# DassHydro-dev/smash

Measured on AMD Instinct MI355X. Metric: cell-timesteps/s, forward+adjoint sweep, higher is better.
Workload: dtype f32

## Files before the change

### __graft_entry__.py

```python
from __future__ import annotations

import os
import subprocess
import sys

ROOT = os.path.dirname(os.path.abspath(__file__))
if ROOT not in sys.path:
    sys.path.insert(0, ROOT)

HIPCC = os.environ.get("HIPCC", "/opt/rocm/bin/hipcc")
CSRC = os.path.join(ROOT, "smash_amd", "csrc")
LIB = os.path.join(ROOT, "smash_amd", "libsmashx.so")
LIB_EXACT = os.path.join(ROOT, "smash_amd", "libsmashx_exact.so")
HIP_FLAGS = ["-O3", "-ffp-contract=off", "--offload-arch=gfx950", "-fPIC", "-shared", "-std=c++17"]


def _newer(target, sources):
    if not os.path.exists(target):
        return False
    t = os.path.getmtime(target)
    return all(os.path.getmtime(s) <= t for s in sources)


def build() -> None:
    srcs = [os.path.join(CSRC, f) for f in sorted(os.listdir(CSRC)) if f.endswith((".hip", ".cpp", ".h"))]
    srcs += [os.path.join(ROOT, "include", "smashx.h"), os.path.join(ROOT, "include", "smashx_setup.h"),
             os.path.join(ROOT, "include", "smashx_forcing.h"), os.path.join(ROOT, "include", "smashx_prcp.h"),
             os.path.join(ROOT, "include", "smashx_signature.h"), os.path.join(ROOT, "include", "smashx_hyper.h"),
             os.path.join(ROOT, "include", "smashx_ann.h"), os.path.join(ROOT, "include", "smashx_sbs.h")]
    jobs = []
    for lib, extra in ((LIB, []), (LIB_EXACT, ["-DSX_EXACT_LIBM=1"])):
        if not _newer(lib, srcs):
            cmd = [HIPCC] + HIP_FLAGS + extra + ["-pthread", "-o", lib, os.path.join(CSRC, "smashx.hip"), os.path.join(CSRC, "sx_plan.cpp"),
                                                 os.path.join(CSRC, "sx_lbfgsb.cpp"), os.path.join(CSRC, "sx_hyper.cpp"), os.path.join(CSRC, "sx_sbs.cpp")]
            jobs.append((cmd, subprocess.Popen(cmd, cwd=ROOT)))
    for cmd, j in jobs:
        if j.wait() != 0:
            raise subprocess.CalledProcessError(j.returncode, cmd)
    subprocess.check_call(["make", "-s", "-C", os.path.join(ROOT, "oracle"), "liboracle.so", "liboracle64.so"])
    ref_src = os.environ.get("SMASH_REFERENCE", "/root/reference")
    ref_lib = os.path.join(ROOT, "oracle", "_ref", "libsmash_ref.so")
    dropin = os.path.join(ROOT, "oracle", "_ref", "libsmash_dropin.so")
    shim = [os.path.join(ROOT, "fortran", "smashx_dropin.f90"), os.path.join(ROOT, "fortran", "smashx_setulb.f90"),
            os.path.join(ROOT, "include", "smashx.h"), os.path.join(ROOT, "oracle", "ref", "ref_capi.f90"),
            os.path.join(ROOT, "oracle", "ref", "build_ref.sh")]
    native_lb = os.path.join(ROOT, "oracle", "_ref", "libsmash_dropin_lbfgsb.so")
    if os.path.isdir(os.path.join(ref_src, "smash", "solver")) and not (os.path.exists(ref_lib) and _newer(dropin, shim) and _newer(native_lb, shim)):
        subprocess.check_call(["bash", os.path.join(ROOT, "oracle", "ref", "build_ref.sh")])
    import smash_amd
    from smash_amd import _lib
    L = _lib.lib()
    missing = [s for s in _lib.SYMBOLS + _lib.SETUP_SYMBOLS + _lib.FORCING_SYMBOLS + _lib.PRCP_SYMBOLS + _lib.SIGNATURE_SYMBOLS + _lib.HYPER_DEVICE_SYMBOLS + _lib.ANN_SYMBOLS + _lib.SBS_SYMBOLS if not hasattr(L, s)]
    if missing:
        raise RuntimeError(f"libsmashx.so lacks {missing}")


def smoke() -> None:
    import numpy as np

    sys.path.insert(0, os.path.join(ROOT, "tests"))
    import golden_util as gu

    import smash_amd
    from oracle import pyoracle
    if not os.path.exists(LIB):
        build()
    g = gu.load("gr_b_16x16x96_nse_gaps")
    ref = pyoracle.run(g.structure, g.mesh, g.dt, g.prcp, g.pet, g.qobs, g.params, g.states, adjoint=True, **g.opts)
    for k, v in g.adj["parameters_b"].items():
        assert np.array_equal(ref["parameters_b"][k], v), k

    setup = smash_amd.SetupDT(0, g.mesh.ng, structure=g.structure, dt=g.dt, ntime_step=g.nt)
    setup.optimize.jobs_fun, setup.optimize.wjobs_fun = ["nse"], [1.0]
    mesh = smash_amd.MeshDT.from_synth(setup, g.mesh)
    inp = smash_amd.Input_DataDT(setup, mesh)
    inp.prcp, inp.pet, inp.qobs = g.prcp, g.pet, g.qobs
    par = smash_amd.ParametersDT.from_dict(mesh, g.params)
    sta = smash_amd.StatesDT.from_dict(mesh, g.states)
    out = smash_amd.OutputDT(setup, mesh)
    par_b, sta_b = par.copy(), sta.copy()
    smash_amd.forward_b(setup, mesh, inp, par, par_b, par.copy(), par.copy(), sta, sta_b, sta.copy(), sta.copy(), out,
                        out.copy(), np.float32(0), np.float32(1))

    errs = {"qsim": (gu.rel_l2(out.qsim, ref["qsim"]), gu.tol(g.noise["qsim"].max())),
            "cost": (abs(out.cost - ref["cost"]), gu.tol_cost(g.noise["cost"], ref["cost"]))}
# ... 15 lines not shown
```

### include/smashx.h

```cpp
#ifndef SMASHX_H
#define SMASHX_H

#ifdef __cplusplus
extern "C" {
#endif

#define SMASHX_GNP 16
#define SMASHX_GNS 8

enum { SMASHX_GR_A = 1, SMASHX_GR_B = 2, SMASHX_GR_C = 3, SMASHX_GR_D = 4, SMASHX_VIC_A = 5 };
enum { SMASHX_NSE = 1, SMASHX_KGE = 2, SMASHX_KGE2 = 3, SMASHX_SE = 4, SMASHX_RMSE = 5, SMASHX_LOGARITHMIC = 6,
       SMASHX_CRC = 7, SMASHX_CFP2 = 8, SMASHX_CFP10 = 9, SMASHX_CFP50 = 10, SMASHX_CFP90 = 11, SMASHX_EPF = 12, SMASHX_ELT = 13,
       SMASHX_ERC = 14 };
enum { SMASHX_PRIOR = 1, SMASHX_SMOOTHING = 2, SMASHX_HARD_SMOOTHING = 3 };
enum { SMASHX_P_CI = 0, SMASHX_P_CP = 1, SMASHX_P_BETA = 2, SMASHX_P_CFT = 3, SMASHX_P_CST = 4, SMASHX_P_ALPHA = 5,
       SMASHX_P_EXC = 6, SMASHX_P_B = 7, SMASHX_P_CUSL1 = 8, SMASHX_P_CUSL2 = 9, SMASHX_P_CLSL = 10, SMASHX_P_KS = 11,
       SMASHX_P_DS = 12, SMASHX_P_DSM = 13, SMASHX_P_WS = 14, SMASHX_P_LR = 15 };
enum { SMASHX_S_HI = 0, SMASHX_S_HP = 1, SMASHX_S_HFT = 2, SMASHX_S_HST = 3, SMASHX_S_HUSL1 = 4, SMASHX_S_HUSL2 = 5,
       SMASHX_S_HLSL = 6, SMASHX_S_HLR = 7 };

enum {
    SMASHX_OK = 0,
    SMASHX_E_ARG = -1,
    SMASHX_E_UNSUPPORTED = -2,
// ... 177 lines not shown
    SMASHX_FN_POW_M025 = 9,
    SMASHX_FN_POW_M025_M125 = 10,
    SMASHX_FN_POW_3P5 = 11,
    SMASHX_FN_POW_3P5_2P5 = 12,
    SMASHX_FN_DIV = 13,
    SMASHX_FN_DIV4 = 14,
    SMASHX_FN_FDIV = 15,
    SMASHX_FN_DIV_FAST = 16,
    SMASHX_FN_COUNT = 17
};
int smashx_selftest_eval(int device, int fn, const float* x, const float* y, long long n, float* out0, float* out1);

#define SMASHX_LBFGSB_START 0
#define SMASHX_LBFGSB_FG 1
#define SMASHX_LBFGSB_NEW_X 2
#define SMASHX_LBFGSB_CONVERGED 3
#define SMASHX_LBFGSB_ABNORMAL 4
typedef struct smashx_lbfgsb smashx_lbfgsb;
int smashx_lbfgsb_create(long n, int m, const double* lower, const double* upper, double factr, double pgtol, smashx_lbfgsb** out);
int smashx_lbfgsb_step(smashx_lbfgsb* opt, double* x, double f, const double* g, int* task);
long smashx_lbfgsb_iterations(const smashx_lbfgsb* opt);
long smashx_lbfgsb_evaluations(const smashx_lbfgsb* opt);
double smashx_lbfgsb_projected_gradient(const smashx_lbfgsb* opt);
const char* smashx_lbfgsb_message(const smashx_lbfgsb* opt);
int smashx_lbfgsb_destroy(smashx_lbfgsb* opt);

#include "smashx_setup.h"
#include "smashx_forcing.h"
#include "smashx_prcp.h"
#include "smashx_signature.h"
#include "smashx_hyper.h"
#include "smashx_ann.h"
#include "smashx_sbs.h"

#ifdef __cplusplus
}
#endif
#endif
```

### smash_amd/_lib.py

```python
from __future__ import annotations

import ctypes as C
import os

_HERE = os.path.dirname(os.path.abspath(__file__))
EXACT = os.environ.get("SMASHX_EXACT_LIBM", "0") not in ("", "0")
LIB_PATH = os.environ.get("SMASHX_LIB", os.path.join(_HERE, "libsmashx_exact.so" if EXACT else "libsmashx.so"))

ABI_VERSION = 9
GNP, GNS = 16, 8
E_OK, E_ARG, E_UNSUPPORTED, E_HIP, E_NODEVICE, E_MESH, E_STATE = 0, -1, -2, -3, -4, -5, -6
STRUCTURES = {"gr-a": 1, "gr-b": 2, "gr-c": 3, "gr-d": 4, "vic-a": 5}
JOBS_FUN = {"nse": 1, "kge": 2, "kge2": 3, "se": 4, "rmse": 5, "logarithmic": 6,
            "Crc": 7, "Cfp2": 8, "Cfp10": 9, "Cfp50": 10, "Cfp90": 11, "Epf": 12, "Elt": 13, "Erc": 14}
SIGNATURE_FUN = ("Crc", "Cfp2", "Cfp10", "Cfp50", "Cfp90", "Epf", "Elt", "Erc")
JREG_FUN = {"prior": 1, "smoothing": 2, "hard_smoothing": 3}
HYPER = {"hyper-linear": 1, "hyper-polynomial": 2}
LBFGSB_START, LBFGSB_FG, LBFGSB_NEW_X, LBFGSB_CONVERGED, LBFGSB_ABNORMAL = range(5)
COMM_ID_BYTES = 128
FN = {k: i for i, k in enumerate("TANH TANH_BRANCHY EXPM1 EXP LOG POW POWB POW_M4 POW_M4_M5 POW_M025 POW_M025_M125 POW_3P5 POW_3P5_2P5 "
                                 "DIV DIV4 FDIV DIV_FAST".split())}
FN_COUNT = len(FN)

HALO_FN = C.CFUNCTYPE(C.c_int, C.c_void_p, C.c_int, C.c_int, C.c_int)
# ... 145 lines not shown
HYPER_DEVICE_SYMBOLS = list(HYPER_DEVICE_PROTOTYPES)
ANN_LAYER = {"dense": 1, "relu": 2, "leaky_relu": 3, "elu": 4, "selu": 5, "sigmoid": 6, "tanh": 7, "scale": 8,
             "softplus": 9, "softmax": 10, "dropout": 11}
_graph = [_int, _int, ptr, ptr, _int]
ANN_PROTOTYPES = {
    "smashx_ann_set_descriptors": (_int, [ptr, _int, ptr]),
    "smashx_ann_set_net": (_int, [ptr, _int, ptr, ptr, _int, ptr, ptr, ptr]),
    "smashx_ann_upload": (_int, [ptr, ptr]),
    "smashx_ann_gradient": (_int, [ptr, ptr]),
    "smashx_ann_fields": (_int, [ptr, _par, _sta]),
    "smashx_ann_info": (_int, [ptr, ptr, ptr]),
    "smashx_ann_host_nweights": (_int, _graph),
    "smashx_ann_host_forward": (_int, _graph + [ptr, ptr, ptr, _long, ptr, ptr]),
    "smashx_ann_host_gradient": (_int, _graph + [ptr, ptr, ptr, _long, ptr, ptr, ptr]),
    "smashx_ann_host_activation": (_int, [_int, _long, ptr, ptr, ptr]),
    "smashx_ann_host_exp": (_int, [_long, ptr, ptr]),
}
ANN_SYMBOLS = list(ANN_PROTOTYPES)
SBS_PROTOTYPES = {
    "smashx_sbs_create": (_int, [_int, ptr, ptr, ptr, _float, _int, _out]),
    "smashx_sbs_ask": (_int, [ptr, ptr, ptr]),
    "smashx_sbs_tell": (_int, [ptr, ptr]),
    "smashx_sbs_x": (_int, [ptr, ptr]),
    "smashx_sbs_gx": (_float, [ptr]),
    "smashx_sbs_ddx": (_float, [ptr]),
    "smashx_sbs_iter": (_int, [ptr]),
    "smashx_sbs_nfg": (_int, [ptr]),
    "smashx_sbs_message": (_str, [ptr]),
    "smashx_sbs_destroy": (_int, [ptr]),
    "smashx_uniform_costs": (_int, [ptr, _par, _sta, _int, ptr, ptr, _int, ptr]),
    "smashx_uniform_costs_info": (_int, [ptr, ptr, ptr]),
}
SBS_SYMBOLS = list(SBS_PROTOTYPES)


class SmashxError(RuntimeError):
    def __init__(self, code, msg):
        super().__init__(f"libsmashx error {code}: {msg}")
        self.code = code


_lib = None


def lib():
    global _lib
    if _lib is None:
        if not os.path.exists(LIB_PATH):
            raise ImportError(f"{LIB_PATH} is missing: build the HIP library first (__graft_entry__.build()); "
                              "smash_amd has no CPU fallback")
        L = C.CDLL(LIB_PATH)
        for name, (restype, argtypes) in list(PROTOTYPES.items()) + list(SETUP_PROTOTYPES.items()) + list(FORCING_PROTOTYPES.items()) + list(PRCP_PROTOTYPES.items()) + list(SIGNATURE_PROTOTYPES.items()) + list(HYPER_DEVICE_PROTOTYPES.items()) + list(ANN_PROTOTYPES.items()) + list(SBS_PROTOTYPES.items()):
            fn = getattr(L, name)
            fn.restype, fn.argtypes = restype, argtypes
        sizes = (C.c_int * 7)()
        L.smashx_abi_sizes(sizes)
        mine = [C.sizeof(t) for t in (Config, Mesh, Options, Parameters, States, Costs, Timing)]
        if list(sizes) != mine:
            raise ImportError(f"{LIB_PATH} was built from another include/smashx.h (struct sizes {list(sizes)}, this module expects {mine}): "
                              "rebuild it (__graft_entry__.build())")
        _lib = L
    return _lib


def check(rc):
    if rc != 0:
        raise SmashxError(rc, lib().smashx_last_error().decode())
```

### smash_amd/csrc/smashx.hip

```cpp
#include "../../include/smashx.h"

#include <hip/hip_runtime.h>
#include <rccl/rccl.h>

#include <dlfcn.h>

#include <algorithm>
#include <functional>
#include <numeric>
#include <cstdio>
#include <cstdlib>
#include <cstring>
#include <string>
#include <vector>

#include "sx_cost.h"
#include "sx_jreg.h"
#include "sx_kernels.h"
#include "sx_ensemble.h"
#include "sx_resident.h"
#include "sx_fields.h"
#include "sx_interception.h"
#include "sx_meanforcing.h"
#include "sx_prcpindices.h"
// ... 248 lines not shown
        if (r_ != ncclSuccess)                                                                          \
            return fail(SMASHX_E_HIP, std::string(#expr) + ": " + rccl().GetErrorString(r_) + " (" + __FILE__ + ":" + std::to_string(__LINE__) + ")"); \
    } while (0)

struct SxComm {
    ncclComm_t comm = nullptr;
    int rank = 0, nranks = 1, device = -1;
    hipStream_t stream = nullptr;
    double* d_buf = nullptr;
    std::vector<smashx_plan*> plans;
};
struct PeerSeg { int rank, first, count; };

struct Launch { hipEvent_t a, b; int kind; double cellsteps; };

}

struct smashx_plan {
    smashx_config cfg{};
    SxSchedule sch;
    int n = 0, npad = 0, nt = 0, ng = 0, st = 0;
    long n2 = 0;
    int M = 0;
    int Tc = 0, nchunks = 0;
    bool have_forcing = false, have_options = false, have_qobs = false, uploaded = false;
    bool chunk_ready = false, adj_ready = false;
    smashx_options opt{};
    std::vector<float> wgauge;
    std::vector<int> gauge_flwacc_h;
    hipStream_t stream = nullptr;
    hipStream_t stream_r = nullptr;
    int Tp = 0;
    bool hi_tape = true;
    int chain_from = 1;
    bool chain_stage = false; SxStageTables stg{}; int stg_blocks = 0, stg_rows_extra = 0; size_t stg_lds = 0;
    float* hrk = nullptr; bool hrk_tried = false, early_adj = true;
    size_t vlds_fwd = 0, vlds_adj = 0;
    std::vector<hipEvent_t> buf_free;
    std::vector<double> round_ncells;
    bool chain_used = false;
    bool chain = true;
    int n_out = 0, n_in = 0;
    int *d_out_x = nullptr, *d_in_x = nullptr;
    float *halo_out = nullptr, *halo_in = nullptr;
    smashx_halo_fn halo_fn = nullptr; void* halo_user = nullptr;
    SxComm* xcomm = nullptr;
    std::vector<PeerSeg> out_segs, in_segs;
    int *d_out_xp = nullptr, *d_in_xp = nullptr;
    float *x_out = nullptr, *x_in = nullptr;
    float* x_keep = nullptr; size_t x_keep_cap = 0;
    std::vector<void*> allocs; std::vector<size_t> alloc_bytes;
    double bytes = 0;
    double hbm_free_at_plan = -1.0, hbm_total = -1.0;
    SxDeviceArrays A{};
    int* d_cell_flat = nullptr;
    int* d_sparse_idx = nullptr;
    float last_jobs_d = 0.f, last_jreg_d = 0.f;
    long n_sparse = 0;
    float* d_stage = nullptr;
    long stage_planes = 0;
    float* d_full[SX_NFIELDS] = {nullptr};
    float* st0[SX_NSSLOTS] = {nullptr};
    float* ckpt = nullptr;
    float* d_prcp = nullptr; float* d_pet = nullptr;
    int* d_ctrl_pos = nullptr; double* d_ctrl = nullptr; size_t ctrl_cap = 0;
    smashx_forcing_layout flay{};
// ... 219 lines not shown
        p->A.hr_rows = Tc / 4;
        p->A.nx = std::max(p->sch.nxslots, 1);
        p->nchunks = (p->nt + Tc - 1) / Tc;
        {
            int want = p->cfg.pipe_steps > 0 ? p->cfg.pipe_steps : Tc;
            const int nsub = std::max(1, (Tc + want / 2) / want);
            p->Tp = std::min(Tc, ((Tc + nsub - 1) / nsub + 15) / 16 * 16);
        }
        int rc;
        if ((rc = p->dmalloc(&p->A.qtT, (size_t)p->npad * Tc))) return rc;
        if ((rc = p->dmalloc(&p->A.xT, (size_t)std::max(p->sch.nxslots, 1) * Tc))) return rc;
        HIPCHK(hipMemsetAsync(p->A.qtT, 0, (size_t)p->npad * Tc * 4, p->stream));
        HIPCHK(hipMemsetAsync(p->A.xT, 0, (size_t)std::max(p->sch.nxslots, 1) * Tc * 4, p->stream));
        p->chunk_ready = true;
    }
    if (p->h_qsim_domain && !p->A.qdT) {
        int rc;
        if ((rc = p->dmalloc(&p->A.qdT, (size_t)p->npad * p->Tc))) return rc;
    }
    if (adjoint && !p->adj_ready) {
        int rc;
        const size_t cs = (size_t)p->npad * p->Tc;
        if (p->A.qsk) { p->dfree(p->A.qsk); p->A.qsk = nullptr; }
        {
            const char* e = getenv("SMASHX_HR_SKEW");
            p->A.hr_skew = e ? atoi(e) != 0 : true;
            if ((rc = p->dmalloc(&p->A.hrT, cs))) return rc;
        }
        if ((rc = p->dmalloc(&p->A.tape_hp, cs))) return rc;
        if ((rc = p->dmalloc(&p->A.tape_hft, cs))) return rc;
        if (st == 5 || ((st == 2 || st == 3) && p->hi_tape)) { if ((rc = p->dmalloc(&p->A.tape_hi, cs))) return rc; }
        else if (st == 2 || st == 3) { if ((rc = p->dmalloc(&p->A.ckpt_hi, cs / SX_HIK))) return rc; }
        if (st == 3) { if ((rc = p->dmalloc(&p->A.tape_hst, cs))) return rc; }
        if (p->nchunks > 1) { if ((rc = p->dmalloc(&p->ckpt, (size_t)p->nchunks * SX_NSSLOTS * p->npad))) return rc; }
        for (int s = 0; s < SX_NSLOTS; ++s) if ((rc = p->dmalloc(&slot_vecs(p, s).grad, (size_t)p->npad))) return rc;
        if ((rc = p->dmalloc(&p->A.qgb, (size_t)std::max(p->ngc, 1) * p->nt))) return rc;
        if ((rc = p->dmalloc(&p->d_qsim_b, (size_t)std::max(p->ng, 1) * p->nt))) return rc;
        p->adj_ready = true;
    }
    if (p->A.ncs > 0 && !p->A.qsk) {
        const size_t need = (size_t)p->A.ncs * 16 * ((size_t)p->Tc / 4 + p->stg_rows_extra + 1);
        size_t fr = 0, tot = 0;
        HIPCHK(hipMemGetInfo(&fr, &tot));
        if ((double)fr > (double)need + 2.0e9) { int rc; if ((rc = p->dmalloc(&p->A.qsk, need / 4))) return rc; }
    }
    if (adjoint && !p->hrk_tried) {
        p->hrk_tried = true;
        const int cf = chain_first(p);
        const char* e = getenv("SMASHX_KEEP_CHAIN_TAPE");
        const bool want = e ? atoi(e) != 0 : true;
        if (const char* ea = getenv("SMASHX_EARLY_ADJ_CHAIN")) p->early_adj = atoi(ea) != 0;
        if (want && p->nchunks > 1 && cf < p->sch.nrounds && !p->tiled && p->n_in == 0 && p->n_out == 0 && p->Tp >= p->Tc) {
            const int kcs0 = p->sch.g_slot_begin[p->sch.round_group_begin[cf]], kncs = p->sch.nslots - kcs0;
            const size_t need = (size_t)(p->nchunks - 1) * (size_t)(p->Tc / 4) * (size_t)kncs * 16;
            size_t fr = 0, tot = 0;
            HIPCHK(hipMemGetInfo(&fr, &tot));
            if (kncs > 0 && (double)fr > (double)need + 2.0e9) {
                int rc; if ((rc = p->dmalloc(&p->hrk, need / 4))) return rc;
                p->A.kcs0 = kcs0; p->A.kncs = kncs;
            }
        }
    }
    return 0;
}

SxDeviceArrays view_at(const smashx_plan* p, int off) {
    SxDeviceArrays B = p->A;
    B.k0 = 0; B.k1 = p->n;
    const size_t q = (size_t)(off / 4);
    B.qtT = p->A.qtT + q * p->npad * 4;
    B.hrk = nullptr;
    if (p->A.hrT) { if (p->A.hr_skew) B.hr_row0 = (int)q; else B.hrT = p->A.hrT + q * p->npad * 4; }
    if (p->A.qdT) B.qdT = p->A.qdT + q * p->npad * 4;
    if (!p->chain) B.qsk = nullptr;
    B.xT = p->A.xT + q * p->A.nx * 4;
    if (p->A.qtdT) B.qtdT = p->A.qtdT + q * p->npad * 4;
    if (p->A.xdT) B.xdT = p->A.xdT + q * p->A.nx * 4;
    if (p->A.tape_hp) B.tape_hp = p->A.tape_hp + (size_t)off * p->npad;
    if (p->A.tape_hft) B.tape_hft = p->A.tape_hft + (size_t)off * p->npad;
    if (p->A.tape_hi) B.tape_hi = p->A.tape_hi + (size_t)off * p->npad;
    if (p->A.ckpt_hi) B.ckpt_hi = p->A.ckpt_hi + (size_t)(off / SX_HIK) * p->npad;
    if (p->A.tape_hst) B.tape_hst = p->A.tape_hst + (size_t)off * p->npad;
    return B;
}

typedef void (*VertKernel)(SxDeviceArrays, int, int);
VertKernel vert_fwd_kernel(int st, bool tape, bool compact) {
#define SX_GR(ST) {sx_k_vert_fwd<ST, false, false>, sx_k_vert_fwd<ST, false, true>, sx_k_vert_fwd<ST, true, false>, sx_k_vert_fwd<ST, true, true>}
    static const VertKernel k[5][4] = {SX_GR(1), SX_GR(2), SX_GR(3), SX_GR(4),
                                       {sx_k_vert_fwd_vic<false, false>, sx_k_vert_fwd_vic<false, true>, sx_k_vert_fwd_vic<true, false>, sx_k_vert_fwd_vic<true, true>}};
#undef SX_GR
    return k[st - 1][2 * tape + compact];
}
VertKernel vert_adj_kernel(int st, bool compact) {
    static const VertKernel k[5][2] = {{sx_k_vert_adj<1, false>, sx_k_vert_adj<1, true>}, {sx_k_vert_adj<2, false>, sx_k_vert_adj<2, true>},
                                       {sx_k_vert_adj<3, false>, sx_k_vert_adj<3, true>}, {sx_k_vert_adj<4, false>, sx_k_vert_adj<4, true>},
                                       {sx_k_vert_adj_vic<false>, sx_k_vert_adj_vic<true>}};
    return k[st - 1][compact];
}
VertKernel vert_tan_kernel(int st) {
    static const VertKernel k[5] = {sx_k_vert_fwd_d<1>, sx_k_vert_fwd_d<2>, sx_k_vert_fwd_d<3>, sx_k_vert_fwd_d<4>, sx_k_vert_fwd_vic_d};
    return k[st - 1];
}
void launch_vert(smashx_plan* p, VertKernel k, int kind, size_t lds, int off, int t0, int T) {
    const SxDeviceArrays B = view_at(p, off);
    if (B.k1 <= B.k0) return;
    const dim3 grid((B.k1 - B.k0 + SX_VBLOCK - 1) / SX_VBLOCK), block(SX_VBLOCK);
    p->mark_begin(kind, p->stream, (double)(B.k1 - B.k0) * T);
    hipLaunchKernelGGL(k, grid, block, lds, p->stream, B, t0, T);
    p->mark_end();
}
void vert_fwd(smashx_plan* p, int off, bool tape, int t0, int T) {
    launch_vert(p, vert_fwd_kernel(p->st, tape, p->A.prcp16 != nullptr), 0, p->st == 5 ? 0 : p->vlds_fwd, off, t0, T);
}
void vert_adj(smashx_plan* p, int off, int t0, int T) {
    launch_vert(p, vert_adj_kernel(p->st, p->A.prcp16 != nullptr), 3, p->st == 5 ? 0 : p->vlds_adj, off, t0, T);
}
void vert_tan(smashx_plan* p, int off, int t0, int T) { launch_vert(p, vert_tan_kernel(p->st), 0, 0, off, t0, T); }
double round_cells(const smashx_plan* p, int r0, int r1) {
    double c = 0.0;
    for (int r = r0; r < r1; ++r) c += p->round_ncells[r];
    return c;
}
int chain_first(const smashx_plan* p) {
    const int nr = p->sch.nrounds;
    return (p->chain && nr - p->chain_from >= 2) ? p->chain_from : nr;
}
void reset_chain_counters(smashx_plan* p, hipStream_t st) {
    (void)hipMemsetAsync(p->A.prog, 0, (size_t)p->sch.ngroups * sizeof(int), st);
    (void)hipMemsetAsync(p->A.prog + p->sch.ngroups + 1, 0, sizeof(int), st);
}
void route_fwd_rounds(smashx_plan* p, int off, bool tape, int t0, int T, hipStream_t st, int r0, int r1, int tan = 0) {
    SxDeviceArrays B = view_at(p, off);
    if (!p->dom_q_active) B.qdT = nullptr;
    if (tan) B.qsk = nullptr;
    const size_t lds = (size_t)2 * p->M * sizeof(float4);
    void (*const k)(SxDeviceArrays, int, int, int, int) = tan == 1 ? sx_k_route_fwd<true, false, 1> : tan == 2 ? sx_k_route_fwd<false, false, 2>
                                                         : tape ? sx_k_route_fwd<true, false> : sx_k_route_fwd<false, false>;
    for (int r = r0; r < r1; ++r) {
        const int g0 = p->sch.round_group_begin[r], ngr = p->sch.round_group_begin[r + 1] - g0;
        p->mark_begin(1, st, round_cells(p, r, r + 1) * T);
        hipLaunchKernelGGL(k, dim3(ngr), dim3(p->M), lds, st, B, g0, g0 + ngr, t0, T);
        p->mark_end();
    }
}
// ... 1358 lines not shown
                                     tiled ? cfg->tile : nullptr, sch, mesh->owner_mask, sublevels_env());
    if (rc) return fail(rc == -5 ? SMASHX_E_MESH : SMASHX_E_ARG, sch.error);
    const int no = (int)sch.out_x.size(), ni = (int)sch.in_x.size();
    const int v[8] = {sch.n, sch.nrounds, sch.ngroups, sch.nslots, sch.nxslots, sch.max_stage, no, ni};
    for (int i = 0; i < 8; ++i) info[i] = v[i];
    if (no > cap || ni > cap) { if (out_src || in_src) return fail(SMASHX_E_ARG, "edge capacity too small"); return 0; }
    for (int i = 0; i < no; ++i) { if (out_src) out_src[i] = sch.out_src[i]; if (out_dst) out_dst[i] = sch.out_dst[i]; }
    for (int i = 0; i < ni; ++i) { if (in_src) in_src[i] = sch.in_src[i]; if (in_dst) in_dst[i] = sch.in_dst[i]; }
    return 0;
}

int smashx_halo_counts(const smashx_plan* p, int* n_out, int* n_in) {
    if (!p || !n_out || !n_in) return fail(SMASHX_E_ARG, "null argument");
    *n_out = p->n_out; *n_in = p->n_in;
    return 0;
}

int smashx_halo_edges(const smashx_plan* p, int* out_src, int* out_dst, int* in_src, int* in_dst) {
    if (!p) return fail(SMASHX_E_ARG, "null plan");
    for (int i = 0; i < p->n_out; ++i) { if (out_src) out_src[i] = p->sch.out_src[i]; if (out_dst) out_dst[i] = p->sch.out_dst[i]; }
    for (int i = 0; i < p->n_in; ++i) { if (in_src) in_src[i] = p->sch.in_src[i]; if (in_dst) in_dst[i] = p->sch.in_dst[i]; }
    return 0;
}

int smashx_plan_chunking(smashx_plan* p, int* chunk_steps, int* pipe_steps) {
    if (!p) return fail(SMASHX_E_ARG, "null plan");
    int rc = set_device(p); if (rc) return rc;
    if ((rc = ensure_chunk_buffers(p, true))) return rc;
    if (chunk_steps) *chunk_steps = p->Tc;
    if (pipe_steps) *pipe_steps = p->Tp;
    return 0;
}

int smashx_plan_hbm(const smashx_plan* p, double out[3]) {
    if (!p || !out) return fail(SMASHX_E_ARG, "null argument");
    out[0] = p->hbm_free_at_plan; out[1] = p->hbm_total; out[2] = p->bytes;
    return 0;
}

int smashx_set_halo(smashx_plan* p, float* d_out_buf, float* d_in_buf, smashx_halo_fn fn, void* user) {
    if (!p) return fail(SMASHX_E_ARG, "null plan");
    if (fn && ((p->n_out > 0 && !d_out_buf) || (p->n_in > 0 && !d_in_buf))) return fail(SMASHX_E_ARG, "halo buffers missing");
    p->halo_out = d_out_buf; p->halo_in = d_in_buf; p->halo_fn = fn; p->halo_user = user;
    return 0;
}

int smashx_set_median_slots(smashx_plan* p, int nslots, const int* slot_of_gauge, smashx_reduce_fn fn, void* user) {
    if (!p || nslots < 0 || (nslots > 0 && !slot_of_gauge)) return fail(SMASHX_E_ARG, "bad argument");
    int rc = set_device(p); if (rc) return rc;
    p->med_nslots = 0; p->med_fn = fn; p->med_user = user;
    if (nslots == 0) return 0;
    std::vector<int> sl(std::max(p->ng, 1), -1);
    for (int g = 0; g < p->ng; ++g) {
        sl[g] = slot_of_gauge[g];
        if (sl[g] < -1 || sl[g] >= nslots) return fail(SMASHX_E_ARG, "slot_of_gauge out of range");
    }
    if (p->have_qobs)
        for (int g = 0; g < p->ng; ++g) {
            if (!(p->wgauge[g] < 0.f) || sl[g] < 0 || gauge_has_data(p, p->h_qobs, g, p->opt.optimize_start_step - 1)) continue;
            return fail(SMASHX_E_UNSUPPORTED, "gauge " + std::to_string(g + 1) + " is given a median slot and has no qobs >= 0 from optimize_start_step on");
        }
    if (p->d_med_slot) { p->dfree(p->d_med_slot); p->dfree(p->d_medx); p->dfree(p->d_medx_idx); }
    if ((rc = p->upload_vec(&p->d_med_slot, sl))) return rc;
    p->med_slot_h = sl;
    if ((rc = p->dmalloc(&p->d_medx, (size_t)3 * nslots))) return rc;
    if ((rc = p->dmalloc(&p->d_medx_idx, (size_t)nslots))) return rc;
// ... 1243 lines not shown
```

### smash_amd/csrc/sx_kernels.h

```cpp
#pragma once

#include <hip/hip_runtime.h>

#include <climits>

#include "sx_ops.h"
#include "sx_tangent.h"
#include "sx_vic.h"

#define SX_BT 4
#define SX_VBLOCK 256

__device__ __forceinline__ void sx_lds_barrier() {
    __builtin_amdgcn_fence(__ATOMIC_RELEASE, "workgroup", "local");
    __builtin_amdgcn_s_barrier();
    __builtin_amdgcn_fence(__ATOMIC_ACQUIRE, "workgroup", "local");
}

__device__ __forceinline__ void sx_lds_wave_fence() {
    __builtin_amdgcn_fence(__ATOMIC_RELEASE, "workgroup", "local");
    __builtin_amdgcn_wave_barrier();
    __builtin_amdgcn_fence(__ATOMIC_ACQUIRE, "workgroup", "local");
}

// ... 80 lines not shown
            }
            __builtin_amdgcn_s_sleep(32);
        }
    }
    __builtin_amdgcn_fence(__ATOMIC_ACQUIRE, "agent");
}
__device__ __forceinline__ void sx_publish(int* prog, int blocks) {
    __builtin_amdgcn_fence(__ATOMIC_RELEASE, "agent");
    __hip_atomic_store((sx_gint*)prog, blocks, __ATOMIC_RELAXED, __HIP_MEMORY_SCOPE_AGENT);
}

struct SxDeviceArrays {
    int n, npad, nt, Tc;
    int k0, k1;
    int nx;
    float dt, dx;
    const float* prcp; const float* pet;
    const unsigned short* prcp16; const float* petd; const float* pet_ratio;
    float prcp_c, prcp_gap; int hour0;
    float *ci, *cp, *cft, *cst, *exc, *lr;
    float* px[3]; float* px_b[3];
    float *rt_a, *rt_f, *rt_denf, *rt_denb;
    int* flwacc;
    float *hi, *hp, *hft, *hst, *hlr;
    float *ci_b, *cp_b, *cft_b, *cst_b, *exc_b, *lr_b, *hi_b, *hp_b, *hft_b, *hst_b, *hlr_b;
    float *qtT, *hrT;
    int hr_skew;
    int hr_rows, hr_row0;
    float* hrk; int kcs0, kncs;
    float *qtdT, *xdT, *qgd;
    float* qdT;
    float *tape_hi, *tape_hp, *tape_hft, *tape_hst;
    float* ckpt_hi;
    float* xT;
    float* qsk; int cs0, ncs;
    float *qg, *qgb;
    int* cell_gauge;
    const int *g_slot_begin, *g_dmax;
    const int *s_cell, *s_stage, *s_sub, *s_wsub, *s_child, *s_ccount, *s_parent, *s_xout;
    const int *x_prod, *x_cons;
    int* prog;
    int ngroups;
    int spin_limit;
    int mute_group;
    long long* gtime;
};

template <class Arrays>
__host__ __device__ __forceinline__ auto& sx_slot_vec(Arrays& A, int slot, bool grad) {
    switch (slot) {
        case SX_SLOT_CI: return grad ? A.ci_b : A.ci;
        case SX_SLOT_CP: return grad ? A.cp_b : A.cp;
        case SX_SLOT_CFT: return grad ? A.cft_b : A.cft;
        case SX_SLOT_CST: return grad ? A.cst_b : A.cst;
        case SX_SLOT_EXC: return grad ? A.exc_b : A.exc;
        case SX_SLOT_LR: return grad ? A.lr_b : A.lr;
        case SX_SLOT_PX0: case SX_SLOT_PX1: case SX_SLOT_PX2: return grad ? A.px_b[slot - SX_SLOT_PX0] : A.px[slot - SX_SLOT_PX0];
        case SX_SLOT_HI: return grad ? A.hi_b : A.hi;
        case SX_SLOT_HP: return grad ? A.hp_b : A.hp;
        case SX_SLOT_HFT: return grad ? A.hft_b : A.hft;
        case SX_SLOT_HST: return grad ? A.hst_b : A.hst;
        default: return grad ? A.hlr_b : A.hlr;
    }
}
template <bool GRAD = false>
struct SxPlanCell {
// ... 160 lines not shown
    template <int S> __device__ __forceinline__ bool no_gap() const {
        if (!COMPACT) return __uint_as_float(p_[S]) >= 0.f && e_[S] >= 0.f;
        return count<S>() != 65535u && __builtin_amdgcn_classf(e_[S], 0x1e0);
    }
    template <int S, bool NOGAP = false> __device__ __forceinline__ float prcp() const {
        if (!COMPACT) return __uint_as_float(p_[S]);
        if (NOGAP) return (float)count<S>() * A.prcp_c;
        return sx_prcp_decode(A, count<S>());
    }
    template <int S, bool NOGAP = false> __device__ __forceinline__ float pet() const {
        if (!COMPACT) return e_[S];
        if (NOGAP) return e_[S] * r_[S];
        return e_[S] < 0.f ? e_[S] : e_[S] * r_[S];
    }
};

template <bool ROW = true, class Cell>
__device__ __forceinline__ void sx_forcing_at(const SxDeviceArrays& A, int t, Cell c, float& p, float& e) {
    const size_t npad = (size_t)A.npad;
    if (A.prcp16 == nullptr) {
        if (ROW) { p = sx_row_load(A.prcp + (size_t)t * npad, c); e = sx_row_load(A.pet + (size_t)t * npad, c); }
        else { p = A.prcp[(size_t)t * npad + c]; e = A.pet[(size_t)t * npad + c]; }
        return;
    }
    p = sx_prcp_decode(A, ROW ? sx_row_load_u16(A.prcp16 + (size_t)t * npad, c >> 1) : (unsigned)A.prcp16[(size_t)t * npad + c]);
    const int q = t + A.hour0;
    const float D = ROW ? sx_row_load(A.petd + (size_t)(q / 24) * npad, c) : A.petd[(size_t)(q / 24) * npad + c];
    e = D < 0.f ? D : D * (ROW ? ((sx_cfloat*)A.pet_ratio)[q % 24] : A.pet_ratio[q % 24]);
}

#ifndef SX_VFWD_WAVES
#define SX_VFWD_WAVES 8
#endif
template <int ST, bool TAPE, bool CF>
#ifndef SX_VFWD_WAVES_GRC
#define SX_VFWD_WAVES_GRC 7
#endif
__global__ __launch_bounds__(SX_VBLOCK, (ST == 2 && CF) ? SX_VFWD_WAVES : (ST == 3 && TAPE && CF) ? SX_VFWD_WAVES_GRC : 1)
void sx_k_vert_fwd(SxDeviceArrays A, int t0, int T) {
    SX_LIBM_INIT();
    const int k = A.k0 + blockIdx.x * SX_VBLOCK + threadIdx.x;
    if (k >= A.k1) return;
    const size_t npad = (size_t)A.npad;

    const SxPlanCell<> cell{A, k};
    SxCellParams P;
    float hi = 0.f, hp = 0.f, hft = 0.f, hst = 0.f;
    sx_cell_params<ST>(cell, P);
    sx_fwd_powers<ST>(P);
    sx_levels_in<ST>(cell, hi, hp, hft, hst);

    const unsigned kb = (unsigned)k * 4u;
    SxForcing<CF> F(A, kb, t0);
    auto step = [&](auto S, int tt) -> float {
        constexpr int s = decltype(S)::value;
        F.template hold<s>();
        if (tt + 1 < T) F.template request<SX_NT, false, 1 - s>(t0 + tt + 1, false);
        if (TAPE) {
            const size_t o = (size_t)tt * npad;
            if (ST == 2 || ST == 3) {
                if (A.tape_hi) sx_row_store<SX_NT>(A.tape_hi + o, kb, hi);
                else if ((tt % SX_HIK) == 0) sx_row_store<SX_NT>(A.ckpt_hi + (size_t)(tt / SX_HIK) * npad, kb, hi);
            }
            sx_row_store<SX_NT>(A.tape_hp + o, kb, hp);
            sx_row_store<SX_NT>(A.tape_hft + o, kb, hft);
            if (ST == 3) sx_row_store<SX_NT>(A.tape_hst + o, kb, hst);
        }
        const float prcp = F.template prcp<s>(), pet = F.template pet<s>();
        const bool still = SX_STILL && sx_wave_all(sx_is_still<ST>(prcp, pet, hi, hp));
        return sx_vertical_step<ST>(P, prcp, pet, hi, hp, hft, hst, still);
    };
    if (T > 0) F.template request<SX_NT, false, 0>(t0, true);
    for (int tq = 0; tq * 4 < T; ++tq) {
        float q[4] = {0.f, 0.f, 0.f, 0.f};
#pragma unroll
        for (int i = 0; i < 4; ++i) {
            const int tt = tq * 4 + i;
            if (tt < T) q[i] = (i & 1) ? step(SxSet<1>{}, tt) : step(SxSet<0>{}, tt);
        }
        sx_row_store4<SX_NT>(A.qtT + (size_t)tq * npad * 4, kb * 4u, q[0], q[1], q[2], q[3]);
    }
    unsigned ke = (unsigned)k;
    sx_pinu(ke);
    sx_levels_out<ST>(SxPlanCell<>{A, (int)ke}, hi, hp, hft, hst);
}

__device__ __forceinline__ SxVicParams sx_vic_load(const SxDeviceArrays& A, int k) {
    return sx_vic_params(SxPlanCell<>{A, k});
}
#ifndef SX_VFWD_WAVES_VIC
#define SX_VFWD_WAVES_VIC 5
#endif
template <bool TAPE, bool CF>
__global__ __launch_bounds__(SX_VBLOCK, TAPE ? SX_VFWD_WAVES_VIC : 1) void sx_k_vert_fwd_vic(SxDeviceArrays A, int t0, int T) {
    SX_LIBM_INIT();
    const int k = A.k0 + blockIdx.x * SX_VBLOCK + threadIdx.x;
    if (k >= A.k1) return;
    const size_t npad = (size_t)A.npad;
    const SxVicParams P = sx_vic_load(A, k);
    const float cusl2_m4 = sx_pow_m4(P.cusl2);
    float husl1 = A.hi[k], husl2 = A.hp[k], hlsl = A.hft[k];
    const unsigned kb = (unsigned)k * 4u;
    SxForcing<CF> F(A, kb, t0);
    if (T > 0) F.template request<SX_NT, false, 1, false>(t0, true);
    for (int tq = 0; tq * 4 < T; ++tq) {
        float q[4] = {0.f, 0.f, 0.f, 0.f};
#pragma unroll
        for (int i = 0; i < 4; ++i) {
            const int tt = tq * 4 + i;
            if (tt < T) {
                F.hold_copy();
                if (tt + 1 < T) F.template request<SX_NT, false, 1, false>(t0 + tt + 1, false);
                if (TAPE) {
// ... 561 lines not shown
#else
#define SX_VADJ_WAVES_GRC 5
#endif
#endif
__global__ __launch_bounds__(SX_VBLOCK, (ST == 2 && CF) ? SX_VADJ_WAVES : (ST == 3 && CF) ? SX_VADJ_WAVES_GRC : 1)
void sx_k_vert_adj(SxDeviceArrays A, int t0, int T) {
    SX_LIBM_INIT();
    const int k = A.k0 + blockIdx.x * SX_VBLOCK + threadIdx.x;
    if (k >= A.k1) return;
    const size_t npad = (size_t)A.npad;
    SxCellParams P;
    sx_cell_params<ST>(SxPlanCell<>{A, k}, P);
    SxAdjParams Q;
    sx_adj_params<ST>(P, Q);
    SxCellGrads G;
    G.ci_b = (ST == 2 || ST == 3) ? A.ci_b[k] : 0.f;
    G.cp_b = A.cp_b[k];
    G.cft_b = A.cft_b[k];
    G.cst_b = (ST == 3) ? A.cst_b[k] : 0.f;
    G.exc_b = (ST != 4) ? A.exc_b[k] : 0.f;
    G.hi_b = (ST == 2 || ST == 3) ? A.hi_b[k] : 0.f;
    G.hp_b = A.hp_b[k];
    G.hft_b = A.hft_b[k];
    G.hst_b = (ST == 3) ? A.hst_b[k] : 0.f;
    const unsigned kb = (unsigned)k * 4u;
    SxForcing<CF> F(A, kb, t0 + T - 1);
    float n_hi[2] = {0.f, 0.f}, n_hp[2] = {0.f, 0.f}, n_hft[2] = {0.f, 0.f}, n_hst[2] = {0.f, 0.f}, n_q[2] = {0.f, 0.f};
    const bool hi_taped = (ST == 2 || ST == 3) && A.tape_hi != nullptr;
    const size_t olast = (size_t)(T > 0 ? T - 1 : 0) * npad;
    const float* r_hi = hi_taped ? A.tape_hi + olast : nullptr;
    const float* r_hp = A.tape_hp + olast;
    const float* r_hft = A.tape_hft + olast;
    const float* r_hst = (ST == 3) ? A.tape_hst + olast : nullptr;
    auto fetch = [&](auto S, int tt, bool first) {
        constexpr int s = decltype(S)::value;
        F.template request<SX_VADJ_NT, true, s>(t0 + tt, first);
        if (hi_taped) { n_hi[s] = sx_row_load<SX_VADJ_NT>(r_hi, kb); r_hi -= npad; }
        n_hp[s] = sx_row_load<SX_VADJ_NT>(r_hp, kb); n_hft[s] = sx_row_load<SX_VADJ_NT>(r_hft, kb);
        r_hp -= npad; r_hft -= npad;
        if (ST == 3) { n_hst[s] = sx_row_load<SX_VADJ_NT>(r_hst, kb); r_hst -= npad; }
        n_q[s] = sx_row_load(A.qtT + (size_t)(tt >> 2) * npad * 4 + (tt & 3), kb * 4u);
    };
    __shared__ float s_hi[(ST == 2 || ST == 3) ? SX_HIK : 1][SX_VBLOCK];
    auto step = [&](auto S, int tt, int tt0) {
        constexpr int s = decltype(S)::value;
        __builtin_amdgcn_sched_barrier(0);
        F.template hold<s>();
        sx_pin1(n_hp[s]); sx_pin1(n_hft[s]); sx_pin1(n_q[s]);
        if (ST == 2 || ST == 3) sx_pin1(n_hi[s]);
        if (ST == 3) sx_pin1(n_hst[s]);
        if (tt > 0) fetch(SxSet<1 - s>{}, tt - 1, false);
        const float hi = (ST == 2 || ST == 3) ? (hi_taped ? n_hi[s] : s_hi[tt - tt0][threadIdx.x]) : 0.f;
        if (SX_GAPFREE && ST == 2 && sx_wave_all(F.template no_gap<s>())) {
            const float prcp = F.template prcp<s, true>(), pet = F.template pet<s, true>();
            const bool still = SX_STILL && sx_wave_all(sx_is_still<ST, true>(prcp, pet, hi, n_hp[s]));
            sx_vertical_step_b<ST, true>(P, Q, prcp, pet, hi, n_hp[s], n_hft[s], n_hst[s], n_q[s], G, still);
            return;
        }
        const float prcp = F.template prcp<s>(), pet = F.template pet<s>();
        const bool still = SX_STILL && sx_wave_all(sx_is_still<ST>(prcp, pet, hi, n_hp[s]));
        sx_vertical_step_b<ST>(P, Q, prcp, pet, hi, n_hp[s], n_hft[s], n_hst[s], n_q[s], G, still);
    };
    if (T > 0) { if ((T - 1) & 1) fetch(SxSet<1>{}, T - 1, true); else fetch(SxSet<0>{}, T - 1, true); }
    for (int tb = (T - 1) / SX_HIK; tb >= 0; --tb) {
        const int tt0 = tb * SX_HIK, len = min(SX_HIK, T - tt0);
        if ((ST == 2 || ST == 3) && !hi_taped) {
            float fp[SX_HIK], fe[SX_HIK];
#pragma unroll
            for (int j = 0; j < SX_HIK; ++j) sx_forcing_at(A, t0 + tt0 + (j < len ? j : 0), kb, fp[j], fe[j]);
            float h = sx_row_load(A.ckpt_hi + (size_t)tb * npad, kb);
#pragma unroll
// ... 24 lines not shown
```

### smash_amd/solver.py

```python
from __future__ import annotations

import ctypes as C

import zlib

import numpy as np

from . import _lib
from ._lib import HYPER, JOBS_FUN, JREG_FUN, SIGNATURE_FUN, STRUCTURES
from .synth import PARAM_DEFAULTS, PARAM_NAMES, STATE_NAMES


RATIO_PET_HOURLY = np.array([0, 0, 0, 0, 0, 0, 0, 0.035, 0.062, 0.079, 0.097, 0.11, 0.117, 0.117, 0.11, 0.097, 0.079, 0.062, 0.035,
                             0, 0, 0, 0, 0], dtype=np.float32)


def _ptr(a):
    return a.ctypes.data_as(C.c_void_p) if a is not None else None


def make_config(setup, mesh, chunk_steps=0, pipe_steps=0, group_size=0, device=-1, tile=None):
    cfg = _lib.Config()
    cfg.structure, cfg.nrow, cfg.ncol = STRUCTURES[setup.structure], mesh.nrow, mesh.ncol
    cfg.nt, cfg.ng, cfg.dt, cfg.dx = setup.ntime_step, mesh.ng, setup.dt, mesh.dx
# ... 165 lines not shown
        def bad(msg):
            return _lib.SmashxError(_lib.E_ARG, "jobs_of_qsim: " + msg)
        for name, a in (("qsim", qsim), ("qsim_d", qsim_d)):
            if a is not None and (not isinstance(a, np.ndarray) or a.shape != (self.ng, self.nt) or a.dtype != np.float32 or not a.flags.f_contiguous):
                raise bad(f"{name} must be a Fortran-ordered float32 array of shape ({self.ng}, {self.nt})")
        if qsim is None:
            raise bad("qsim is None")
        qb = np.zeros((self.ng, self.nt), np.float32, order="F") if jobs_b is not None else None
        jobs, jobs_d = C.c_float(0.0), C.c_float(0.0)
        _lib.check(_lib.lib().smashx_jobs_of_qsim(self._h, _ptr(qsim), float(jobs_b or 0.0), C.byref(jobs), _ptr(qb), _ptr(qsim_d),
                                                  C.byref(jobs_d) if qsim_d is not None else None))
        return np.float32(jobs.value), qb, (np.float32(jobs_d.value) if qsim_d is not None else None)

    def halo_counts(self):
        a, b = C.c_int(0), C.c_int(0)
        _lib.check(_lib.lib().smashx_halo_counts(self._h, C.byref(a), C.byref(b)))
        return a.value, b.value

    def halo_edges(self):
        no, ni = self.halo_counts()
        arr = [np.zeros(max(n, 1), np.int32) for n in (no, no, ni, ni)]
        _lib.check(_lib.lib().smashx_halo_edges(self._h, *[_ptr(a) for a in arr]))
        return arr[0][:no], arr[1][:no], arr[2][:ni], arr[3][:ni]

    def chunking(self):
        a, b = C.c_int(0), C.c_int(0)
        _lib.check(_lib.lib().smashx_plan_chunking(self._h, C.byref(a), C.byref(b)))
        return a.value, b.value

    def hbm(self):
        v = (C.c_double * 3)()
        _lib.check(_lib.lib().smashx_plan_hbm(self._h, v))
        return {"free_at_plan": v[0], "total": v[1], "held": v[2]}

    def set_domain_outputs(self, qsim_domain=None, net_prcp_domain=None, sparse=False):
        for a in (qsim_domain, net_prcp_domain):
            if a is not None and not (a.dtype == np.float32 and a.flags.f_contiguous):
                raise _lib.SmashxError(_lib.E_ARG, "domain outputs must be Fortran-ordered float32 arrays")
        self._dom_keep = (qsim_domain, net_prcp_domain)
        _lib.check(_lib.lib().smashx_set_domain_outputs(self._h, _ptr(qsim_domain), _ptr(net_prcp_domain), bool(sparse)))

    def tangent_terms(self):
        a, b = C.c_float(0.0), C.c_float(0.0)
        _lib.check(_lib.lib().smashx_tangent_terms(self._h, C.byref(a), C.byref(b)))
        return float(a.value), float(b.value)

    def group_times(self):
        ng = self.timing()["n_groups"]
        out = np.zeros((2, ng, 2), np.int64)
        rnd = np.zeros(ng, np.int32)
        _lib.check(_lib.lib().smashx_debug_group_times(self._h, _ptr(out), _ptr(rnd)))
        return out, rnd

    def set_halo(self, out_ptr, in_ptr, fn):
        def tramp(user, phase, t0, nsteps):
            try:
                return int(fn(phase, t0, nsteps) or 0)
            except Exception:
                import traceback
                traceback.print_exc()
                return 1
        self._halo_cb = _lib.HALO_FN(tramp)
        _lib.check(_lib.lib().smashx_set_halo(self._h, out_ptr, in_ptr, self._halo_cb, None))

    def set_median_slots(self, nslots, slot_of_gauge, reduce_fn=None):
        sl = np.ascontiguousarray(slot_of_gauge, np.int32) if self.ng else np.full(1, -1, np.int32)
# ... 719 lines not shown
```

Before: 57.14 billion.

## Skip taping unchanged hi/hp rows per wavefront and reuse them in adjoint

In the taped forward pass for GR-B with compact forcing, each wavefront now checks whether the interception and production states are bitwise unchanged across a step. When they are, it skips storing that tape row and sets a bit in a per-wave flag word, written once every 16 steps. The adjoint reads these flags and reuses the previous register value instead of loading the row from memory. The aim is to cut tape write and read traffic when states are static, such as on dry steps, at the cost of extra flag memory, wave-wide votes and more complex fetch logic. An env variable and a debug API report the skip counts.

```diff
diff --git a/__graft_entry__.py b/__graft_entry__.py
--- a/__graft_entry__.py
+++ b/__graft_entry__.py
@@ -27,7 +27,8 @@
     srcs += [os.path.join(ROOT, "include", "smashx.h"), os.path.join(ROOT, "include", "smashx_setup.h"),
              os.path.join(ROOT, "include", "smashx_forcing.h"), os.path.join(ROOT, "include", "smashx_prcp.h"),
              os.path.join(ROOT, "include", "smashx_signature.h"), os.path.join(ROOT, "include", "smashx_hyper.h"),
-             os.path.join(ROOT, "include", "smashx_ann.h"), os.path.join(ROOT, "include", "smashx_sbs.h")]
+             os.path.join(ROOT, "include", "smashx_ann.h"), os.path.join(ROOT, "include", "smashx_sbs.h"),
+             os.path.join(ROOT, "include", "smashx_tape.h")]
     jobs = []
     for lib, extra in ((LIB, []), (LIB_EXACT, ["-DSX_EXACT_LIBM=1"])):
         if not _newer(lib, srcs):
@@ -50,7 +51,7 @@
     import smash_amd
     from smash_amd import _lib
     L = _lib.lib()
-    missing = [s for s in _lib.SYMBOLS + _lib.SETUP_SYMBOLS + _lib.FORCING_SYMBOLS + _lib.PRCP_SYMBOLS + _lib.SIGNATURE_SYMBOLS + _lib.HYPER_DEVICE_SYMBOLS + _lib.ANN_SYMBOLS + _lib.SBS_SYMBOLS if not hasattr(L, s)]
+    missing = [s for s in _lib.SYMBOLS + _lib.SETUP_SYMBOLS + _lib.FORCING_SYMBOLS + _lib.PRCP_SYMBOLS + _lib.SIGNATURE_SYMBOLS + _lib.HYPER_DEVICE_SYMBOLS + _lib.ANN_SYMBOLS + _lib.SBS_SYMBOLS + _lib.TAPE_SYMBOLS if not hasattr(L, s)]
     if missing:
         raise RuntimeError(f"libsmashx.so lacks {missing}")
 
diff --git a/include/smashx.h b/include/smashx.h
--- a/include/smashx.h
+++ b/include/smashx.h
@@ -233,6 +233,7 @@
 #include "smashx_hyper.h"
 #include "smashx_ann.h"
 #include "smashx_sbs.h"
+#include "smashx_tape.h"
 
 #ifdef __cplusplus
 }
diff --git a/include/smashx_tape.h b/include/smashx_tape.h
--- /dev/null
+++ b/include/smashx_tape.h
@@ -0,0 +1,15 @@
+#ifndef SMASHX_TAPE_H
+#define SMASHX_TAPE_H
+
+#include "smashx.h"
+
+#ifdef __cplusplus
+extern "C" {
+#endif
+
+int smashx_plan_tape_skip(smashx_plan* plan, long long* out);
+
+#ifdef __cplusplus
+}
+#endif
+#endif
diff --git a/smash_amd/_lib.py b/smash_amd/_lib.py
--- a/smash_amd/_lib.py
+++ b/smash_amd/_lib.py
@@ -201,6 +201,10 @@
     "smashx_uniform_costs_info": (_int, [ptr, ptr, ptr]),
 }
 SBS_SYMBOLS = list(SBS_PROTOTYPES)
+TAPE_PROTOTYPES = {
+    "smashx_plan_tape_skip": (_int, [ptr, ptr]),
+}
+TAPE_SYMBOLS = list(TAPE_PROTOTYPES)
 
 
 class SmashxError(RuntimeError):
@@ -219,7 +223,7 @@
             raise ImportError(f"{LIB_PATH} is missing: build the HIP library first (__graft_entry__.build()); "
                               "smash_amd has no CPU fallback")
         L = C.CDLL(LIB_PATH)
-        for name, (restype, argtypes) in list(PROTOTYPES.items()) + list(SETUP_PROTOTYPES.items()) + list(FORCING_PROTOTYPES.items()) + list(PRCP_PROTOTYPES.items()) + list(SIGNATURE_PROTOTYPES.items()) + list(HYPER_DEVICE_PROTOTYPES.items()) + list(ANN_PROTOTYPES.items()) + list(SBS_PROTOTYPES.items()):
+        for name, (restype, argtypes) in list(PROTOTYPES.items()) + list(SETUP_PROTOTYPES.items()) + list(FORCING_PROTOTYPES.items()) + list(PRCP_PROTOTYPES.items()) + list(SIGNATURE_PROTOTYPES.items()) + list(HYPER_DEVICE_PROTOTYPES.items()) + list(ANN_PROTOTYPES.items()) + list(SBS_PROTOTYPES.items()) + list(TAPE_PROTOTYPES.items()):
             fn = getattr(L, name)
             fn.restype, fn.argtypes = restype, argtypes
         sizes = (C.c_int * 7)()
diff --git a/smash_amd/csrc/smashx.hip b/smash_amd/csrc/smashx.hip
--- a/smash_amd/csrc/smashx.hip
+++ b/smash_amd/csrc/smashx.hip
@@ -304,6 +304,7 @@
     hipStream_t stream_r = nullptr;
     int Tp = 0;
     bool hi_tape = true;
+    bool tape_skip = true; int skip_off = -1, skip_T = 0;
     int chain_from = 1;
     bool chain_stage = false; SxStageTables stg{}; int stg_blocks = 0, stg_rows_extra = 0; size_t stg_lds = 0;
     float* hrk = nullptr; bool hrk_tried = false, early_adj = true;
@@ -589,6 +590,16 @@
         if (st == 5 || ((st == 2 || st == 3) && p->hi_tape)) { if ((rc = p->dmalloc(&p->A.tape_hi, cs))) return rc; }
         else if (st == 2 || st == 3) { if ((rc = p->dmalloc(&p->A.ckpt_hi, cs / SX_HIK))) return rc; }
         if (st == 3) { if ((rc = p->dmalloc(&p->A.tape_hst, cs))) return rc; }
+        if (sx_tape_skip(st, true) || sx_tape_skip(st, false)) {
+            if (const char* e = getenv("SMASHX_TAPE_SKIP")) p->tape_skip = atoi(e) != 0;
+            p->A.nwaves = (p->npad + 63) / 64;
+            p->A.tape_all = p->tape_skip ? 0 : 1;
+            const size_t fw = (size_t)(p->Tc / 16) * p->A.nwaves;
+            if ((rc = p->dmalloc(&p->A.flag_hp, fw))) return rc;
+            if ((rc = p->dmalloc(&p->A.flag_hi, fw))) return rc;
+            HIPCHK(hipMemsetAsync(p->A.flag_hp, 0, fw * 4, p->stream));
+            HIPCHK(hipMemsetAsync(p->A.flag_hi, 0, fw * 4, p->stream));
+        }
         if (p->nchunks > 1) { if ((rc = p->dmalloc(&p->ckpt, (size_t)p->nchunks * SX_NSSLOTS * p->npad))) return rc; }
         for (int s = 0; s < SX_NSLOTS; ++s) if ((rc = p->dmalloc(&slot_vecs(p, s).grad, (size_t)p->npad))) return rc;
         if ((rc = p->dmalloc(&p->A.qgb, (size_t)std::max(p->ngc, 1) * p->nt))) return rc;
@@ -638,6 +649,7 @@
     if (p->A.tape_hi) B.tape_hi = p->A.tape_hi + (size_t)off * p->npad;
     if (p->A.ckpt_hi) B.ckpt_hi = p->A.ckpt_hi + (size_t)(off / SX_HIK) * p->npad;
     if (p->A.tape_hst) B.tape_hst = p->A.tape_hst + (size_t)off * p->npad;
+    if (p->A.flag_hp) { B.flag_hp = p->A.flag_hp + (size_t)(off / 16) * p->A.nwaves; B.flag_hi = p->A.flag_hi + (size_t)(off / 16) * p->A.nwaves; }
     return B;
 }
 
@@ -668,6 +680,7 @@
     p->mark_end();
 }
 void vert_fwd(smashx_plan* p, int off, bool tape, int t0, int T) {
+    if (tape) { p->skip_off = off; p->skip_T = T; }
     launch_vert(p, vert_fwd_kernel(p->st, tape, p->A.prcp16 != nullptr), 0, p->st == 5 ? 0 : p->vlds_fwd, off, t0, T);
 }
 void vert_adj(smashx_plan* p, int off, int t0, int T) {
@@ -2092,6 +2105,25 @@
     return 0;
 }
 
+int smashx_plan_tape_skip(smashx_plan* p, long long* out) {
+    if (!p || !out) return fail(SMASHX_E_ARG, "null argument");
+    if (!p->adj_ready || p->skip_off < 0) return fail(SMASHX_E_STATE, "smashx_plan_tape_skip: no taped forward launch has run");
+    int rc = set_device(p); if (rc) return rc;
+    const int nw = (p->n + 63) / 64, nb = (p->skip_T + 15) / 16;
+    out[0] = out[1] = 0; out[2] = p->skip_T; out[3] = nw;
+    if (!sx_tape_skip(p->st, p->A.prcp16 != nullptr) || nb == 0) return 0;
+    HIPCHK(hipStreamSynchronize(p->stream));
+    std::vector<unsigned> w((size_t)nb * p->A.nwaves);
+    const unsigned* src[2] = {p->A.tape_hi ? p->A.flag_hi : nullptr, p->A.flag_hp};
+    for (int l = 0; l < 2; ++l) {
+        if (!src[l]) continue;
+        HIPCHK(hipMemcpy(w.data(), src[l] + (size_t)(p->skip_off / 16) * p->A.nwaves, w.size() * 4, hipMemcpyDeviceToHost));
+        for (int b = 0; b < nb; ++b)
+            for (int v = 0; v < nw; ++v) out[l] += __builtin_popcount(w[(size_t)b * p->A.nwaves + v]);
+    }
+    return 0;
+}
+
 int smashx_plan_hbm(const smashx_plan* p, double out[3]) {
     if (!p || !out) return fail(SMASHX_E_ARG, "null argument");
     out[0] = p->hbm_free_at_plan; out[1] = p->hbm_total; out[2] = p->bytes;
diff --git a/smash_amd/csrc/sx_kernels.h b/smash_amd/csrc/sx_kernels.h
--- a/smash_amd/csrc/sx_kernels.h
+++ b/smash_amd/csrc/sx_kernels.h
@@ -136,6 +136,7 @@
     float* qdT;
     float *tape_hi, *tape_hp, *tape_hft, *tape_hst;
     float* ckpt_hi;
+    unsigned *flag_hi, *flag_hp; int nwaves, tape_all;
     float* xT;
     float* qsk; int cs0, ncs;
     float *qg, *qgb;
@@ -362,6 +363,14 @@
 #ifndef SX_VFWD_WAVES
 #define SX_VFWD_WAVES 8
 #endif
+#ifndef SX_TAPE_SKIP
+#define SX_TAPE_SKIP 1
+#endif
+#ifndef SX_TAPE_SKIP_ALL
+#define SX_TAPE_SKIP_ALL 0
+#endif
+constexpr bool sx_tape_skip(int st, bool compact) { return SX_TAPE_SKIP && (SX_TAPE_SKIP_ALL ? st <= 4 : (st == 2 && compact)); }
+typedef const __attribute__((address_space(4))) unsigned sx_cuint;
 template <int ST, bool TAPE, bool CF>
 #ifndef SX_VFWD_WAVES_GRC
 #define SX_VFWD_WAVES_GRC 7
@@ -382,23 +391,37 @@
 
     const unsigned kb = (unsigned)k * 4u;
     SxForcing<CF> F(A, kb, t0);
+    constexpr bool SKIP = TAPE && sx_tape_skip(ST, CF);
+    unsigned f_hi = 0u, f_hp = 0u;
     auto step = [&](auto S, int tt) -> float {
         constexpr int s = decltype(S)::value;
         F.template hold<s>();
         if (tt + 1 < T) F.template request<SX_NT, false, 1 - s>(t0 + tt + 1, false);
+        const size_t o = (size_t)tt * npad;
         if (TAPE) {
-            const size_t o = (size_t)tt * npad;
             if (ST == 2 || ST == 3) {
-                if (A.tape_hi) sx_row_store<SX_NT>(A.tape_hi + o, kb, hi);
+                if (A.tape_hi) { if (!SKIP) sx_row_store<SX_NT>(A.tape_hi + o, kb, hi); }
                 else if ((tt % SX_HIK) == 0) sx_row_store<SX_NT>(A.ckpt_hi + (size_t)(tt / SX_HIK) * npad, kb, hi);
             }
-            sx_row_store<SX_NT>(A.tape_hp + o, kb, hp);
+            if (!SKIP) sx_row_store<SX_NT>(A.tape_hp + o, kb, hp);
             sx_row_store<SX_NT>(A.tape_hft + o, kb, hft);
             if (ST == 3) sx_row_store<SX_NT>(A.tape_hst + o, kb, hst);
         }
         const float prcp = F.template prcp<s>(), pet = F.template pet<s>();
         const bool still = SX_STILL && sx_wave_all(sx_is_still<ST>(prcp, pet, hi, hp));
-        return sx_vertical_step<ST>(P, prcp, pet, hi, hp, hft, hst, still);
+        if (!SKIP) return sx_vertical_step<ST>(P, prcp, pet, hi, hp, hft, hst, still);
+        const float hi0 = hi, hp0 = hp;
+        const float q = sx_vertical_step<ST>(P, prcp, pet, hi, hp, hft, hst, still);
+        const bool keep = (tt == T - 1) | (A.tape_all != 0);
+        if (A.tape_hi) {
+            const bool same = sx_wave_all(__float_as_uint(hi0) == __float_as_uint(hi)) && !keep;
+            if (!same) sx_row_store<SX_NT>(A.tape_hi + o, kb, hi0);
+            f_hi |= (same ? 1u : 0u) << (tt & 15);
+        }
+        const bool same = sx_wave_all(__float_as_uint(hp0) == __float_as_uint(hp)) && !keep;
+        if (!same) sx_row_store<SX_NT>(A.tape_hp + o, kb, hp0);
+        f_hp |= (same ? 1u : 0u) << (tt & 15);
+        return q;
     };
     if (T > 0) F.template request<SX_NT, false, 0>(t0, true);
     for (int tq = 0; tq * 4 < T; ++tq) {
@@ -409,6 +432,15 @@
             if (tt < T) q[i] = (i & 1) ? step(SxSet<1>{}, tt) : step(SxSet<0>{}, tt);
         }
         sx_row_store4<SX_NT>(A.qtT + (size_t)tq * npad * 4, kb * 4u, q[0], q[1], q[2], q[3]);
+        if (SKIP && ((tq & 3) == 3 || tq * 4 + 4 >= T)) {
+            if ((threadIdx.x & 63u) == 0u) {
+                const size_t w = (size_t)(tq >> 2) * (size_t)A.nwaves;
+                const unsigned wb = (kb >> 6) & ~3u;
+                if (A.tape_hi) sx_row_store((float*)(A.flag_hi + w), wb, __uint_as_float(f_hi));
+                sx_row_store((float*)(A.flag_hp + w), wb, __uint_as_float(f_hp));
+            }
+            f_hi = 0u; f_hp = 0u;
+        }
     }
     unsigned ke = (unsigned)k;
     sx_pinu(ke);
@@ -1036,11 +1068,37 @@
     const float* r_hp = A.tape_hp + olast;
     const float* r_hft = A.tape_hft + olast;
     const float* r_hst = (ST == 3) ? A.tape_hst + olast : nullptr;
+    constexpr bool SKIP = sx_tape_skip(ST, CF);
+    unsigned w_hi = 0u, w_hp = 0u, wn_hi = 0u, wn_hp = 0u;
+    sx_cuint* fl_hi = nullptr; sx_cuint* fl_hp = nullptr;
+    const size_t nwaves = (size_t)A.nwaves;
+    if (SKIP && T >= 2) {
+        const int wv = __builtin_amdgcn_readfirstlane(k >> 6);
+        fl_hp = (sx_cuint*)A.flag_hp + wv;
+        wn_hp = fl_hp[(size_t)((T - 2) >> 4) * nwaves];
+        if (hi_taped) { fl_hi = (sx_cuint*)A.flag_hi + wv; wn_hi = fl_hi[(size_t)((T - 2) >> 4) * nwaves]; }
+    }
     auto fetch = [&](auto S, int tt, bool first) {
         constexpr int s = decltype(S)::value;
         F.template request<SX_VADJ_NT, true, s>(t0 + tt, first);
-        if (hi_taped) { n_hi[s] = sx_row_load<SX_VADJ_NT>(r_hi, kb); r_hi -= npad; }
-        n_hp[s] = sx_row_load<SX_VADJ_NT>(r_hp, kb); n_hft[s] = sx_row_load<SX_VADJ_NT>(r_hft, kb);
+        bool c_hi = false, c_hp = false;
+        if (SKIP && !first) {
+            if ((tt & 15) == 15 || tt == T - 2) {
+                w_hi = wn_hi; w_hp = wn_hp;
+                if (tt >= 16) {
+                    const size_t b = (size_t)((tt >> 4) - 1) * nwaves;
+                    wn_hp = fl_hp[b];
+                    if (hi_taped) wn_hi = fl_hi[b];
+                }
+            }
+            c_hi = ((w_hi >> (tt & 15)) & 1u) != 0u; c_hp = ((w_hp >> (tt & 15)) & 1u) != 0u;
+        }
+        if (hi_taped) {
+            if (c_hi) n_hi[s] = n_hi[1 - s]; else n_hi[s] = sx_row_load<SX_VADJ_NT>(r_hi, kb);
+            r_hi -= npad;
+        }
+        if (c_hp) n_hp[s] = n_hp[1 - s]; else n_hp[s] = sx_row_load<SX_VADJ_NT>(r_hp, kb);
+        n_hft[s] = sx_row_load<SX_VADJ_NT>(r_hft, kb);
         r_hp -= npad; r_hft -= npad;
         if (ST == 3) { n_hst[s] = sx_row_load<SX_VADJ_NT>(r_hst, kb); r_hst -= npad; }
         n_q[s] = sx_row_load(A.qtT + (size_t)(tt >> 2) * npad * 4 + (tt & 3), kb * 4u);
diff --git a/smash_amd/solver.py b/smash_amd/solver.py
--- a/smash_amd/solver.py
+++ b/smash_amd/solver.py
@@ -221,6 +221,11 @@
         v = (C.c_double * 3)()
         _lib.check(_lib.lib().smashx_plan_hbm(self._h, v))
         return {"free_at_plan": v[0], "total": v[1], "held": v[2]}
+
+    def tape_skip(self):
+        v = (C.c_longlong * 4)()
+        _lib.check(_lib.lib().smashx_plan_tape_skip(self._h, v))
+        return {"hi_rows": int(v[0]), "hp_rows": int(v[1]), "steps": int(v[2]), "wavefronts": int(v[3])}
 
     def set_domain_outputs(self, qsim_domain=None, net_prcp_domain=None, sparse=False):
         for a in (qsim_domain, net_prcp_domain):
```

Result: no change. 57.62 billion, median of 6 (+0.8%).
